# sta105/VIORB

Measured on AMD Instinct MI355X. Metric: frames/sec ORB extract+match+pose-opt, EuRoC 752x480, 1/2/4/8 GPUs, higher is better.
Workload: dtype u8

## Files before the change

### viorb_amd/csrc/orb_extractor.hip

```cpp
#include <hip/hip_runtime.h>
#include <stdlib.h>
#include <math.h>
#include <vector>
#include <string>
#include <algorithm>
#include "viorb_common.h"
#include "orb_math.h"
#include "octree_arrays.h"

namespace viorb {

static const int8_t kPatternHost[1024] = {
#include "orb_pattern.inc"
};

enum { MINB = 16, PATCH = 31, HALF_PATCH = 15, MAX_LEVELS = 16 };

struct LevelDev {
    int w, h, stride;
    uint32_t plane_off;
    int cell_base, ncells;
    int quota;
    int oct_w, oct_h;
    int n_ini;
// ... 151 lines not shown
    uint32_t v[RS2_TRIPS]; int at[RS2_TRIPS], gr[RS2_TRIPS], gc[RS2_TRIPS];
#pragma unroll
    for (int k = 0; k < RS2_TRIPS; k++) {
        const int i = threadIdx.x + 256 * k, ic = min(i, total - 1);
        const int r = ic / A.lds_pitch_dw, c = ic - r * A.lds_pitch_dw;
        at[k] = (i < total && c < ndw) ? i : -1;
        gr[k] = ys0 + r; gc[k] = xs0 + 4 * min(c, ndw - 1);
        v[k] = *reinterpret_cast<const uint32_t*>(src + (size_t)gr[k] * A.src_stride + gc[k]);
    }
    if (threadIdx.x < RS2_TW) s_xt[threadIdx.x] = tab; else if (threadIdx.x < RS2_TW + RS2_TH) s_yt[threadIdx.x - RS2_TW] = tab;
#pragma unroll
    for (int k = 0; k < RS2_TRIPS; k++) if (at[k] >= 0) s_tile[at[k]] = v[k];
    if (A.copy_dst) {
        uint8_t* cd = A.copy_dst + (size_t)b * A.copy_pitch;
#pragma unroll
        for (int k = 0; k < RS2_TRIPS; k++) if (at[k] >= 0) *reinterpret_cast<uint32_t*>(cd + (size_t)gr[k] * A.copy_stride + gc[k]) = v[k];
    }
    __syncthreads();
    const uint8_t* t8 = reinterpret_cast<const uint8_t*>(s_tile);
    const int xg = threadIdx.x & 15, r0 = threadIdx.x >> 4;
    int2 xt[4];
#pragma unroll
    for (int j = 0; j < 4; j++) xt[j] = s_xt[xg * 4 + j];
    uint8_t* dst = A.dst + (size_t)b * A.dst_pitch;
    const int pitch = A.lds_pitch_dw * 4;
#pragma unroll
    for (int half = 0; half < 2; half++) {
        const int r = r0 + 16 * half, dy = ty0 + r;
        if (dy >= A.dst_h) continue;
        const int2 yt = s_yt[r];
        const uint8_t* S0 = t8 + ((yt.x & 0xffff) - ys0) * pitch - xs0;
        const uint8_t* S1 = t8 + ((yt.x >> 16) - ys0) * pitch - xs0;
        const int b0 = yt.y & 0xffff, b1 = yt.y >> 16;
        uint32_t packed = 0;
#pragma unroll
        for (int j = 0; j < 4; j++) {
            const int sx0 = xt[j].x & 0xffff, sx1 = xt[j].x >> 16, a0 = xt[j].y & 0xffff, a1 = xt[j].y >> 16;
            const int h0 = S0[sx0] * a0 + S0[sx1] * a1;
            const int h1 = S1[sx0] * a0 + S1[sx1] * a1;
            const int val = (((b0 * (h0 >> 4)) >> 16) + ((b1 * (h1 >> 4)) >> 16) + 2) >> 2;
            packed |= (uint32_t)(val & 0xff) << (8 * j);
        }
        const int dxw = tx0 + xg * 4;
        if (dxw < A.dst_stride) *reinterpret_cast<uint32_t*>(dst + (size_t)dy * A.dst_stride + dxw) = packed;
    }
}

typedef unsigned short ushort2v __attribute__((ext_vector_type(2)));
__device__ __forceinline__ uint32_t dot2_u16(uint32_t a, uint32_t k, uint32_t c) {
    return __builtin_amdgcn_udot2(__builtin_bit_cast(ushort2v, a), __builtin_bit_cast(ushort2v, k), c, false);
}
#define RSS_LANES 32
#define RSS_PF 6
#define RSS_MAX_SRC_ROWS 60
struct ResizeStreamArgs {
    const uint8_t* planes; size_t frame_bytes;
    uint32_t src_off, dst_off;
    int src_stride, src_h, dst_stride, dst_w, dst_h;
    const int2* xtab; const int2* ytab; const uint2* etab; const int4* items;
};
struct __attribute__((packed, aligned(1))) rss_u8x8 { uint32_t lo, hi; };
__global__ __launch_bounds__(64) void k_resize_stream(ResizeStreamArgs A, XcdPlace PL) {
    int b, item;
    if (!xcd_place(PL, b, item)) return;
    const int4 t = A.items[item];
    const uint8_t* src = A.planes + (size_t)b * A.frame_bytes + A.src_off;
    uint8_t* dst = const_cast<uint8_t*>(A.planes) + (size_t)b * A.frame_bytes + A.dst_off;
    const int lane = threadIdx.x, hl = lane & (RSS_LANES - 1);
    const bool upper = lane >= RSS_LANES;
    const int Rb = t.z, y0A = t.y, y0B = t.y + Rb;
    const int rowsA = min(Rb, A.dst_h - y0A), rowsB = max(min(Rb, A.dst_h - y0B), 0);
    const int rsA = A.ytab[y0A].x & 0xffff, reA = A.ytab[y0A + rowsA - 1].x >> 16;
    const int rsB = rowsB > 0 ? A.ytab[min(y0B, A.dst_h - 1)].x & 0xffff : 0, reB = rowsB > 0 ? A.ytab[min(y0B + rowsB - 1, A.dst_h - 1)].x >> 16 : -1;
    const int ns = max(reA - rsA, reB - rsB) + 1;
    const int d = t.x + hl, sdw = A.dst_stride >> 2;
    uint32_t sel[4], aw[4]; int sxf = 0;
#pragma unroll
    for (int j = 0; j < 4; j++) {
        const int2 e = A.xtab[min(4 * d + j, A.dst_w - 1)];
        if (j == 0) sxf = e.x & 0xffff;
        sel[j] = (uint32_t)((e.x & 0xffff) - sxf) | ((uint32_t)((e.x >> 16) - sxf) << 16) | 0x0c000c00u;
        aw[j] = (uint32_t)e.y;
    }
    auto pack_entry = [&](int r0, int r1, int yb0, int nrows) {
        const int r = r0 + lane;
        const uint2 e = A.etab[min(r, A.src_h - 1)];
        const int y = (int)(e.x & 0x7fff) - yb0;
        const bool ok = r <= r1 && (e.x & 0x7fff) != 0x7fff && y >= 0 && y < nrows;
        return ok ? ((uint32_t)y | ((e.y & 0xfffu) << 7) | (((e.y >> 16) & 0xfffu) << 19) | ((e.x >> 15) << 31)) : 127u;
    };
    const uint32_t EA = pack_entry(rsA, reA, y0A, rowsA), EB = pack_entry(rsB, reB, y0B, rowsB);
    const uint8_t* pc = src + sxf;
    uint8_t* pd = dst + 4u * (uint32_t)min(d, sdw - 1);
    const bool col_ok = d < sdw;
    uint32_t lo[RSS_PF], hi[RSS_PF];
    auto request = [&](int i, uint32_t& l, uint32_t& h) {
        const uint32_t offA = __builtin_amdgcn_readfirstlane(min(rsA + i, A.src_h - 1) * A.src_stride), offB = __builtin_amdgcn_readfirstlane(min(rsB + i, A.src_h - 1) * A.src_stride);
        const rss_u8x8 v = *reinterpret_cast<const rss_u8x8*>(pc + (upper ? offB : offA));
        l = v.lo; h = v.hi;
    };
#pragma unroll
    for (int u = 0; u < RSS_PF; u++) request(u, lo[u], hi[u]);
    uint32_t hp[4] = {0, 0, 0, 0};
    for (int i0 = 0; i0 < ns; i0 += RSS_PF) {
#pragma unroll
        for (int u = 0; u < RSS_PF; u++) {
            const int i = i0 + u;
            uint32_t hc[4];
#pragma unroll
            for (int j = 0; j < 4; j++) {
                const uint32_t two = __builtin_amdgcn_perm(hi[u], lo[u], sel[j]);
                hc[j] = (dot2_u16(two, aw[j], 0u) & 0x7fff0u) << 5;
            }
            request(i + RSS_PF, lo[u], hi[u]);
            const uint32_t eA = __builtin_amdgcn_readlane(EA, i & 63), eB = __builtin_amdgcn_readlane(EB, i & 63);
            const uint32_t yrA = eA & 127u, yrB = eB & 127u;
            const bool emit = upper ? yrB < (uint32_t)rowsB : yrA < (uint32_t)rowsA;
            if (emit && col_ok) {
                const uint32_t b0 = upper ? (eB & (0xfffu << 7)) : (eA & (0xfffu << 7)), b1 = upper ? ((eB >> 12) & (0xfffu << 7)) : ((eA >> 12) & (0xfffu << 7));
                const uint32_t yoA = __builtin_amdgcn_readfirstlane((y0A + (int)yrA) * A.dst_stride), yoB = __builtin_amdgcn_readfirstlane((y0B + (int)yrB) * A.dst_stride);
                const uint32_t yo = upper ? yoB : yoA;
                uint32_t h0[4] = {hp[0], hp[1], hp[2], hp[3]};
                if ((int)(eA | eB) < 0) {
                    const bool same = upper ? (int)eB < 0 : (int)eA < 0;
#pragma unroll
                    for (int j = 0; j < 4; j++) h0[j] = same ? hc[j] : hp[j];
                }
                uint32_t v[4];
#pragma unroll
                for (int j = 0; j < 4; j++) {
                    const uint32_t t0 = (uint32_t)(((unsigned long long)h0[j] * b0) >> 32), t1 = (uint32_t)(((unsigned long long)hc[j] * b1) >> 32);
                    v[j] = (t0 + t1 + 2u) >> 2;
                }
                const uint32_t w01 = v[0] | (v[1] << 8), w23 = v[2] | (v[3] << 8);
                *reinterpret_cast<uint32_t*>(pd + yo) = w01 | (w23 << 16);
            }
#pragma unroll
            for (int j = 0; j < 4; j++) hp[j] = hc[j];
        }
    }
}

typedef short short2v __attribute__((ext_vector_type(2)));
__device__ __forceinline__ uint32_t pk_min16(uint32_t a, uint32_t b) {
    return __builtin_bit_cast(uint32_t, __builtin_elementwise_min(__builtin_bit_cast(short2v, a), __builtin_bit_cast(short2v, b)));
}
__device__ __forceinline__ uint32_t pk_max16(uint32_t a, uint32_t b) {
    return __builtin_bit_cast(uint32_t, __builtin_elementwise_max(__builtin_bit_cast(short2v, a), __builtin_bit_cast(short2v, b)));
}
__device__ __forceinline__ uint32_t pk_sub16(uint32_t a, uint32_t b) {
    return __builtin_bit_cast(uint32_t, __builtin_bit_cast(short2v, a) - __builtin_bit_cast(short2v, b));
}
__device__ __forceinline__ uint32_t swap16(uint32_t a) { return __builtin_amdgcn_alignbit(a, a, 16); }
__device__ __forceinline__ int fast_strength(const uint8_t* p, int pitch) {
    const uint32_t v = p[0], vv = v | (v << 16);
    uint32_t P[8];
    P[0] = pk_sub16(vv, (uint32_t)p[3 * pitch] | ((uint32_t)p[-3 * pitch] << 16));
    P[1] = pk_sub16(vv, (uint32_t)p[3 * pitch + 1] | ((uint32_t)p[-3 * pitch - 1] << 16));
    P[2] = pk_sub16(vv, (uint32_t)p[2 * pitch + 2] | ((uint32_t)p[-2 * pitch - 2] << 16));
    P[3] = pk_sub16(vv, (uint32_t)p[pitch + 3] | ((uint32_t)p[-pitch - 3] << 16));
    P[4] = pk_sub16(vv, (uint32_t)p[3] | ((uint32_t)p[-3] << 16));
    P[5] = pk_sub16(vv, (uint32_t)p[-pitch + 3] | ((uint32_t)p[pitch - 3] << 16));
    P[6] = pk_sub16(vv, (uint32_t)p[-2 * pitch + 2] | ((uint32_t)p[2 * pitch - 2] << 16));
    P[7] = pk_sub16(vv, (uint32_t)p[-3 * pitch + 1] | ((uint32_t)p[3 * pitch - 1] << 16));
    uint32_t S[8], lo2[8], hi2[8], lo4[8], hi4[8];
#pragma unroll
    for (int k = 0; k < 8; k++) S[k] = swap16(P[k]);
#pragma unroll
    for (int k = 0; k < 8; k++) { const uint32_t nx = k < 7 ? P[k + 1] : S[0]; lo2[k] = pk_min16(P[k], nx); hi2[k] = pk_max16(P[k], nx); }
#pragma unroll
    for (int k = 0; k < 8; k++) {
        const uint32_t nl = k < 6 ? lo2[k + 2] : swap16(lo2[k - 6]), nh = k < 6 ? hi2[k + 2] : swap16(hi2[k - 6]);
        lo4[k] = pk_min16(lo2[k], nl); hi4[k] = pk_max16(hi2[k], nh);
    }
    uint32_t A = 0x80008000u, B = 0x7fff7fffu;
#pragma unroll
    for (int k = 0; k < 8; k++) {
        const uint32_t nl = k < 4 ? lo4[k + 4] : swap16(lo4[k - 4]), nh = k < 4 ? hi4[k + 4] : swap16(hi4[k - 4]);
        A = pk_max16(A, pk_min16(pk_min16(lo4[k], nl), S[k]));
        B = pk_min16(B, pk_max16(pk_max16(hi4[k], nh), S[k]));
    }
    const int a = max((int)(short)(A & 0xffff), (int)(short)(A >> 16)), bq = min((int)(short)(B & 0xffff), (int)(short)(B >> 16));
    return max(a, -bq) - 1;
}

__device__ __forceinline__ int wave_inclusive_scan(int v) {
    v += __builtin_amdgcn_update_dpp(0, v, 0x111, 0xf, 0xf, false);
    v += __builtin_amdgcn_update_dpp(0, v, 0x112, 0xf, 0xf, false);
    v += __builtin_amdgcn_update_dpp(0, v, 0x114, 0xf, 0xf, false);
    v += __builtin_amdgcn_update_dpp(0, v, 0x118, 0xf, 0xf, false);
    v += __builtin_amdgcn_update_dpp(0, v, 0x142, 0xa, 0xf, false);
    v += __builtin_amdgcn_update_dpp(0, v, 0x143, 0xc, 0xf, false);
    return v;
}
__constant__ uint32_t c_rcp16[64];
#define FAST_FETCH_TRIPS 7
#define FAST_LAUNCHES 8
#define FAST_CELLS_PER_WAVE 2
__global__ __launch_bounds__(64) void k_fast_cells(const uint8_t* __restrict__ planes, size_t frame_bytes,
                                                   const LevelDev* __restrict__ lv,
                                                   const CellDesc* __restrict__ cells, int ini_th, int min_th,
                                                   uint32_t* __restrict__ slots, int slot_cap,
                                                   int* __restrict__ cell_cnt, int ncells_total,
                                                   int tile_bytes, int score_bytes, int list_cap, XcdPlace PL) {
    extern __shared__ uint32_t s_mem[];
    int img_b, item;
    if (!xcd_place(PL, img_b, item)) return;
    uint8_t* tile = reinterpret_cast<uint8_t*>(s_mem);
    uint8_t* sc = tile + tile_bytes;
    uint16_t* surv = reinterpret_cast<uint16_t*>(sc + score_bytes);
    uint16_t* corn = surv + list_cap;
    const int lane = threadIdx.x;
    const int cell0 = item * FAST_CELLS_PER_WAVE;
    const int ncell = min((int)FAST_CELLS_PER_WAVE, ncells_total - cell0);
    uint32_t v[FAST_FETCH_TRIPS];
    const uint8_t* img = planes + (size_t)img_b * frame_bytes;
    auto request_tile = [&](const CellDesc& cd) {
        const int pdw = cd.pitch >> 2;
// ... 748 lines not shown
            finish = true;
        } else if (live + n_to_expand * 3 > N) {
            int guard2 = 0;
            while (!finish && guard2++ < 4096) {
                const int prev2 = live;
                int m = 0;
                for (int base = first_new; base < nn; base += 64) {
                    const int i = base + lane;
                    bool want = false; SortKey key = 0;
                    if (i < nn) { const Node o = S.nd[i]; want = o.count > 1; key = ((SortKey)o.count << OctT<BIG>::KEY_SHIFT) | (SortKey)i; }
                    const unsigned long long bm = __ballot(want);
                    if (want) { const int pos = m + __popcll(bm & lanemask_lt(lane)); if (pos < sortcap) S.sortb[pos] = key; }
                    m += __popcll(bm);
                }
                if (m > sortcap) { overflow = true; m = sortcap; }
                int mp = 1; while (mp < m) mp <<= 1;
                for (int i = m + lane; i < mp; i += 64) S.sortb[i] = 0;
                WAVE_SYNC();
                oct_sort(S.sortb, mp, lane);
                const int nn1 = nn;
                int processed = 0;
                bool reached = false;
                for (int base = 0; base < m && !reached && !finish; base += 64) {
                    const int q = base + lane;
                    const bool valid = q < m;
                    const int i = valid ? (int)(S.sortb[mp - 1 - q] & 0xffff) : 0;
                    Node p; p.flags = OCT_DEAD; p.count = 0;
                    if (valid) p = S.nd[i];
                    if (__any(valid && p.count > OCT_LANE_LIMIT)) {
                        for (int l = 0; l < 64 && base + l < m; l++) {
                            if (nn1 + 4 * (processed + 1) > nodecap) { overflow = true; finish = true; break; }
                            const OctExpandResult r = oct_expand_wave(S, (int)(S.sortb[mp - 1 - (base + l)] & 0xffff), nn1 + 4 * processed, lane);
                            processed++; live += r.off - 1;
                            if (live >= N) { reached = true; break; }
                        }
                        continue;
                    }
                    const int mx = p.x0 + ((p.x1 - p.x0 + 1) >> 1), my = p.y0 + ((p.y1 - p.y0 + 1) >> 1);
                    unsigned long long lo = 0, hi = 0; int tc[4] = {0, 0, 0, 0};
                    if (valid) oct_lane_count(S, p, mx, my, lo, hi, tc);
                    const int inc = valid ? (tc[0] > 0) + (tc[1] > 0) + (tc[2] > 0) + (tc[3] > 0) - 1 : 0;
                    const int incl = wave_inclusive_scan(inc);
                    const unsigned long long mh = __ballot(valid && live + incl >= N);
                    const int nvalid = min(64, m - base);
                    int cut = mh ? __ffsll((long long)mh) - 1 : nvalid - 1;
                    const int fit = (nodecap - nn1) / 4 - processed;
                    if (fit < cut + 1) { overflow = true; finish = true; cut = fit - 1; }
                    if (valid && lane <= cut) oct_lane_scatter(S, p, i, nn1 + 4 * (processed + lane), mx, my, lo, hi, tc);
                    if (cut >= 0) { live += __shfl(incl, cut); processed += cut + 1; }
                    if (mh) reached = true;
                }
                nn = nn1 + 4 * processed;
                WAVE_SYNC();
                nn = oct_compact(S, nn, nn1, lane, first_new);
                if (live >= N || live == prev2) finish = true;
            }
        }
    }
    if (defer_nodes && overflow) {
        if (lane == 0) lvl_tot[b * nlevels + level] |= 0x40000000;
        return;
    }
    for (int base = 0; base < nn; base += 64) {
        const int i = base + lane;
        if (i < nn) {
            const Node o = S.nd[i];
            const Perm* pm = (o.flags & OCT_BUF) ? S.perm1 : S.perm0;
            uint32_t best = S.keys[pm[o.begin]];
            for (int k = 1; k < (int)o.count; k++) {
                const uint32_t key = S.keys[pm[o.begin + k]];
                if ((key >> 24) > (best >> 24)) best = key;
            }
            out[nn - 1 - i] = (best & 0xff000000u) | ((((best >> 12) & 0xfff) + MINB) << 12) | ((best & 0xfff) + MINB);
        }
    }
    if (lane == 0) {
        lvl_cnt[b * nlevels + level] = nn;
        if (overflow) status[b] = VIORB_ERR_CAPACITY;
    }
}

#define BS_LANES 32
#define BS_PF 6
__constant__ int c_gauss[7];
__global__ __launch_bounds__(64) void k_blur(const uint8_t* __restrict__ planes, uint8_t* __restrict__ blur,
                                             size_t frame_bytes, const LevelDev* __restrict__ lv,
                                             const int4* __restrict__ items, XcdPlace PL) {
    int b, item;
    if (!xcd_place(PL, b, item)) return;
    const int4 t = items[item];
    const LevelDev L = lv[t.x];
    const uint8_t* src = planes + (size_t)b * frame_bytes + L.plane_off;
    uint8_t* dst = blur + (size_t)b * frame_bytes + L.plane_off;
    const int lane = threadIdx.x, hl = lane & (BS_LANES - 1);
    const bool upper = lane >= BS_LANES;
    const int Rb = t.w, y0A = t.z, y0B = t.z + Rb;
    const int rows = upper ? min(Rb, L.h - y0B) : min(Rb, L.h - y0A);
    const int sdw = L.stride >> 2;
    const int d = t.y + hl;
    const int dlast = (L.w - 1) >> 2, m = (L.w - 1) & 3;
    const int dc = min(d, sdw - 1);
    const bool end_lane = hl == 0 || hl == BS_LANES - 1;
    const int dn = hl == 0 ? max(dc - 1, 0) : min(dc + 1, sdw - 1);
    const uint32_t selC = m == 0 ? 0x01020304u : m == 1 ? 0x03040504u : m == 2 ? 0x05060504u : 0x07060504u;
    const uint32_t selR = m == 0 ? 0x0c0c0c0cu : m == 1 ? 0x0c000102u : m == 2 ? 0x01020304u : 0x03040506u;
    const bool has_edge = t.y == 0 || t.y + BS_LANES > dlast - 1;
    const bool is_d0 = d == 0, is_dl = d == dlast, is_dl1 = d == dlast - 1;
    const uint32_t k0 = (uint32_t)c_gauss[0], k1 = (uint32_t)c_gauss[1], k2 = (uint32_t)c_gauss[2], k3 = (uint32_t)c_gauss[3];
    const uint32_t Ka = k0 | (k1 << 8) | (k2 << 16) | (k3 << 24), Kb = k2 | (k1 << 8) | (k0 << 16);
    const uint32_t K01 = k0 | (k1 << 16), K23 = k2 | (k3 << 16), K45 = k2 | (k1 << 16);
    const int nrow = Rb + 6;
    const uint8_t* pc = src + 4u * (uint32_t)dc;
    const uint8_t* pn = src + 4u * (uint32_t)(end_lane ? dn : dc);
    uint32_t cb[BS_PF], nb[BS_PF];
    auto request = [&](int i, uint32_t& c, uint32_t& n) {
        const int ii = min(i, nrow - 1);
        int ya = y0A + ii - 3, yb = y0B + ii - 3;
        ya = ya < 0 ? -ya : ya; ya = ya >= L.h ? 2 * L.h - 2 - ya : ya; ya = min(max(ya, 0), L.h - 1);
        yb = yb < 0 ? -yb : yb; yb = yb >= L.h ? 2 * L.h - 2 - yb : yb; yb = min(max(yb, 0), L.h - 1);
        const uint32_t offA = __builtin_amdgcn_readfirstlane(ya * L.stride), offB = __builtin_amdgcn_readfirstlane(yb * L.stride);
        const uint32_t off = upper ? offB : offA;
        c = *reinterpret_cast<const uint32_t*>(pc + off);
        n = *reinterpret_cast<const uint32_t*>(pn + off);
    };
#pragma unroll
    for (int u = 0; u < BS_PF; u++) request(u, cb[u], nb[u]);
    uint32_t P[6][4], hp[4] = {0, 0, 0, 0};
#pragma unroll
    for (int u = 0; u < 6; u++) { P[u][0] = P[u][1] = P[u][2] = P[u][3] = 0; }
    uint8_t* pd = dst + 4u * (uint32_t)min(d, sdw - 1);
    const bool col_ok = d < sdw;
    for (int i0 = 0; i0 < nrow; i0 += 6) {
#pragma unroll
        for (int u = 0; u < 6; u++) {
            const int i = i0 + u;
            uint32_t c = cb[u];
            uint32_t Lr = __builtin_amdgcn_update_dpp(c, c, 0x138, 0xf, 0xf, true);
            uint32_t Rr = __builtin_amdgcn_update_dpp(c, c, 0x130, 0xf, 0xf, true);
            Lr = hl == 0 ? nb[u] : Lr; Rr = hl == BS_LANES - 1 ? nb[u] : Rr;
            request(i + BS_PF, cb[u], nb[u]);
            if (has_edge) {
                const uint32_t Lf = __builtin_amdgcn_perm(Rr, c, 0x01020304u);
                const uint32_t Cf = __builtin_amdgcn_perm(c, Lr, selC), Rf = __builtin_amdgcn_perm(c, Lr, selR);
                const uint32_t Rf1 = __builtin_amdgcn_perm(Rr, c, selC);
                Lr = is_d0 ? Lf : Lr;
                Rr = is_dl ? Rf : (is_dl1 ? Rf1 : Rr);
                c = is_dl ? Cf : c;
            }
            uint32_t h[4];
            h[0] = __builtin_amdgcn_udot4(__builtin_amdgcn_alignbyte(c, Lr, 1), Ka, __builtin_amdgcn_udot4(__builtin_amdgcn_alignbyte(Rr, c, 1), Kb, 0u, false), false);
            h[1] = __builtin_amdgcn_udot4(__builtin_amdgcn_alignbyte(c, Lr, 2), Ka, __builtin_amdgcn_udot4(__builtin_amdgcn_alignbyte(Rr, c, 2), Kb, 0u, false), false);
            h[2] = __builtin_amdgcn_udot4(__builtin_amdgcn_alignbyte(c, Lr, 3), Ka, __builtin_amdgcn_udot4(__builtin_amdgcn_alignbyte(Rr, c, 3), Kb, 0u, false), false);
            h[3] = __builtin_amdgcn_udot4(c, Ka, __builtin_amdgcn_udot4(Rr, Kb, 0u, false), false);
            uint32_t a[4];
#pragma unroll
            for (int j = 0; j < 4; j++) {
                a[j] = dot2_u16(P[(u + 1) % 6][j], K01, 1u << 15);
                a[j] = dot2_u16(P[(u + 3) % 6][j], K23, a[j]);
                a[j] = dot2_u16(P[(u + 5) % 6][j], K45, a[j]);
                a[j] = __umul24(h[j], k0) + a[j];
                a[j] = min(a[j], 0x00ffffffu);
                P[u][j] = hp[j] | (h[j] << 16);
                hp[j] = h[j];
            }
            const int o = i - 6;
            const uint32_t yoA = __builtin_amdgcn_readfirstlane((y0A + o) * L.stride), yoB = __builtin_amdgcn_readfirstlane((y0B + o) * L.stride);
            if (o >= 0 && o < rows && col_ok) {
                const uint32_t lo = __builtin_amdgcn_perm(a[1], a[0], 0x0c0c0602u), hi = __builtin_amdgcn_perm(a[3], a[2], 0x0c0c0602u);
                *reinterpret_cast<uint32_t*>(pd + (upper ? yoB : yoA)) = lo | (hi << 16);
            }
        }
    }
}

__constant__ __attribute__((aligned(16))) uint32_t c_pattern[256];
__constant__ int c_umax[16];
__constant__ uint32_t c_orient_mask[256];
typedef uint32_t u32_unaligned __attribute__((aligned(1)));
#define DESC_WIN_HALF 18
#define DESC_WIN_ROWS 37
#define DESC_WIN_DW 10
#define DESC_WIN_TRIPS 6
__global__ __launch_bounds__(256) void k_orient_describe(const uint8_t* __restrict__ planes,
                                                         const uint8_t* __restrict__ blur, size_t frame_bytes,
                                                         const LevelDev* __restrict__ lv, int nlevels,
                                                         const uint32_t* __restrict__ lvl_kp, int kp_pitch,
                                                         const int* __restrict__ lvl_cnt,
                                                         viorb_keypoint* __restrict__ out_kp,
                                                         uint8_t* __restrict__ out_desc, int out_cap,
                                                         int* __restrict__ out_cnt, int* __restrict__ status, XcdPlace PL) {
    const int lane = threadIdx.x & 63;
    int b, item;
    if (!xcd_place(PL, b, item)) return;
    const int k = item * 4 + __builtin_amdgcn_readfirstlane(threadIdx.x >> 6);
    const int* cnt = lvl_cnt + b * nlevels;
    int level = -1, local = 0, total = 0;
    for (int l = 0; l < nlevels; l++) {
        const int c = cnt[l];
        if (level < 0 && k < total + c) { level = l; local = k - total; }
        total += c;
    }
    if (k == 0 && lane == 0) { out_cnt[b] = min(total, out_cap); if (total > out_cap) status[b] = VIORB_ERR_CAPACITY; }
    if (level < 0 || k >= out_cap) return;
    const LevelDev L = lv[level];
    const uint32_t key = lvl_kp[(size_t)b * kp_pitch + L.kp_off + local];
    const int cx = (int)(key & 0xfff), cy = (int)((key >> 12) & 0xfff), score = (int)(key >> 24);
    const uint8_t* img = planes + (size_t)b * frame_bytes + L.plane_off + (size_t)cy * L.stride + cx;
    __shared__ uint32_t s_win[4][DESC_WIN_ROWS * DESC_WIN_DW];
    uint32_t* win = s_win[threadIdx.x >> 6];
    const uint8_t* bim = blur + (size_t)b * frame_bytes + L.plane_off + (size_t)cy * L.stride + cx;
    uint32_t wv[DESC_WIN_TRIPS];
#pragma unroll
    for (int it = 0; it < DESC_WIN_TRIPS; it++) {
        const int i = min(lane + 64 * it, DESC_WIN_ROWS * DESC_WIN_DW - 1);
        const int wr = i / DESC_WIN_DW, wc = i - wr * DESC_WIN_DW;
        wv[it] = *reinterpret_cast<const u32_unaligned*>(bim + __mul24(wr - DESC_WIN_HALF, L.stride) - DESC_WIN_HALF + 4 * wc);
    }
    int m10 = 0, m01 = 0;
    {
        const int j = lane & 7, r8 = lane >> 3;
        const uint32_t wu = 0x03020100u + 0x04040404u * (uint32_t)j;
        const uint8_t* col = img - HALF_PATCH + 4 * j;
        uint32_t px[4]; int vv[4];
#pragma unroll
        for (int it = 0; it < 4; it++) {
            const int row = min(it * 8 + r8, PATCH - 1);
            vv[it] = row - HALF_PATCH;
            px[it] = *reinterpret_cast<const u32_unaligned*>(col + __mul24(vv[it], L.stride));
        }
#pragma unroll
        for (int it = 0; it < 4; it++) {
            const uint32_t q = px[it] & c_orient_mask[it * 64 + lane];
            const int s1 = (int)__builtin_amdgcn_udot4(q, 0x01010101u, 0u, false);
            const int su = (int)__builtin_amdgcn_udot4(q, wu, 0u, false);
            m10 += su - __mul24(HALF_PATCH, s1);
            m01 += __mul24(vv[it], s1);
        }
    }
    m10 = __builtin_amdgcn_readlane(wave_inclusive_scan(m10), 63); m01 = __builtin_amdgcn_readlane(wave_inclusive_scan(m01), 63);
    const float angle = fast_atan2_deg((float)m01, (float)m10);
    const float factor_pi = (float)(3.14159265358979323846 / 180.f);
    float sn, cs;
    sincos_f32(angle * factor_pi, &sn, &cs);
    const float a = cs, bb = sn;
#pragma unroll
    for (int it = 0; it < DESC_WIN_TRIPS; it++) {
        const int i = lane + 64 * it;
        if (i < DESC_WIN_ROWS * DESC_WIN_DW) win[i] = wv[it];
    }
    __builtin_amdgcn_fence(__ATOMIC_RELEASE, "wavefront"); __builtin_amdgcn_wave_barrier(); __builtin_amdgcn_fence(__ATOMIC_ACQUIRE, "wavefront");
    const uint8_t* w8 = reinterpret_cast<const uint8_t*>(win) + DESC_WIN_HALF * (DESC_WIN_DW * 4) + DESC_WIN_HALF;
    uint32_t nib = 0;
// ... 292 lines not shown
                    c.src_off = (uint32_t)(L.plane_off + (size_t)c.y0 * L.stride + (size_t)(c.x0 & ~3)); c.stride = L.stride;
                    if (c.cw < 7 || c.ch < 7) continue;
                    h->cells.push_back(c);
                    max_cw = std::max(max_cw, (int)c.cw); max_ch = std::max(max_ch, (int)c.ch);
                }
            }
        }
        L.ncells = (int)h->cells.size() - L.cell_base;
        L.n_ini = (L.oct_h > 0 && L.oct_w > 0) ? (int)roundf((float)L.oct_w / (float)L.oct_h) : 0;
        L.hx = L.n_ini > 0 ? (float)L.oct_w / (float)L.n_ini : 1.f;
        L.kp_off = kp_off;
        kp_off += std::max(L.quota, 4 * L.n_ini) + 4;
        L.xtab_off = (int)xtab.size(); L.ytab_off = (int)ytab.size();
        if (l > 0) {
            const int sw = h->lv[l - 1].w, sh = h->lv[l - 1].h;
            const double inv_sx = (double)L.w / sw, inv_sy = (double)L.h / sh;
            const double scale_x = 1. / inv_sx, scale_y = 1. / inv_sy;
            for (int dx = 0; dx < L.w; dx++) {
                float fx = (float)((dx + 0.5) * scale_x - 0.5);
                int sx = host_cv_floor(fx);
                fx -= sx;
                if (sx < 0) { fx = 0; sx = 0; }
                if (sx + 1 >= sw && sx >= sw - 1) { fx = 0; sx = sw - 1; }
                const int a0 = clampi(host_cv_round((double)((1.f - fx) * 2048)), -32768, 32767);
                const int a1 = clampi(host_cv_round((double)(fx * 2048)), -32768, 32767);
                const int sx1 = std::min(sx + 1, sw - 1);
                xtab.push_back(make_int2(sx | (sx1 << 16), (a0 & 0xffff) | (a1 << 16)));
            }
            for (int dy = 0; dy < L.h; dy++) {
                float fy = (float)((dy + 0.5) * scale_y - 0.5);
                int sy = host_cv_floor(fy);
                fy -= sy;
                const int b0 = clampi(host_cv_round((double)((1.f - fy) * 2048)), -32768, 32767);
                const int b1 = clampi(host_cv_round((double)(fy * 2048)), -32768, 32767);
                const int sy0 = clampi(sy, 0, sh - 1), sy1 = clampi(sy + 1, 0, sh - 1);
                ytab.push_back(make_int2(sy0 | (sy1 << 16), (b0 & 0xffff) | (b1 << 16)));
            }
            int maxdw = 1, maxrows = 1;
            const int2* xt = xtab.data() + L.xtab_off; const int2* yt = ytab.data() + L.ytab_off;
            for (int tx = 0; tx < L.w; tx += RS_TW) {
                const int x1 = std::min(tx + RS_TW, L.w) - 1;
                const int xs0 = (xt[tx].x & 0xffff) & ~3, xs1 = xt[x1].x >> 16;
                maxdw = std::max(maxdw, ((xs1 - xs0) >> 2) + 1);
            }
            for (int ty = 0; ty < L.h; ty += RS_TH) {
                const int y1 = std::min(ty + RS_TH, L.h) - 1;
                maxrows = std::max(maxrows, (yt[y1].x >> 16) - (yt[ty].x & 0xffff) + 1);
            }
            h->rs_pitch_dw[l] = maxdw; h->rs_rows[l] = maxrows;
            if ((size_t)maxdw * maxrows * 4 > 60000) { set_error("resize tile does not fit LDS (scale factor too large)"); return VIORB_ERR_UNSUPPORTED; }
            {
                h->rs2_off[l] = (int)h->rs2_tiles.size();
                int pdw = 1, prow = 1; bool cover = true; int next_x = 0, next_y = 0;
                const int gx2 = (L.w + RS2_TW - 1) / RS2_TW, gy2 = (L.h + RS2_TH - 1) / RS2_TH;
                for (int ty = 0; ty < gy2; ty++) {
                    const int y0t = ty * RS2_TH, y1t = std::min(y0t + RS2_TH, L.h) - 1;
                    const int ys0 = yt[y0t].x & 0xffff, ys1 = yt[y1t].x >> 16;
                    if (ys0 > next_y) cover = false;
                    next_y = std::max(next_y, ys1 + 1);
                    next_x = 0;
                    for (int tx = 0; tx < gx2; tx++) {
                        const int x0t = tx * RS2_TW, x1t = std::min(x0t + RS2_TW, L.w) - 1;
                        const int xs0 = (xt[x0t].x & 0xffff) & ~3, xs1 = xt[x1t].x >> 16;
                        if (xs0 > next_x) cover = false;
                        next_x = std::max(next_x, (xs1 | 3) + 1);
                        const int ndw = ((xs1 - xs0) >> 2) + 1, nrows = ys1 - ys0 + 1;
                        pdw = std::max(pdw, ndw); prow = std::max(prow, nrows);
                        h->rs2_tiles.push_back(make_int4(xs0, ndw, ys0, nrows));
                    }
                    if (next_x < sw) cover = false;
                }
                if (next_y < sh) cover = false;
                h->rs2_pitch_dw[l] = pdw;
                h->rs2_ok[l] = (prow <= 48 && pdw * prow <= 256 * RS2_TRIPS) ? 1 : 0;
                if (l == 1) h->rs2_copy_ok = cover && h->rs2_ok[1];
            }
            {
                static const bool no_stream = getenv("VIORB_RESIZE_TILES") != nullptr;
                bool ok = !no_stream && sw >= 8;
                h->rss_etab_off[l] = (int)h->rss_etab.size();
                std::vector<uint2> et(sh, make_uint2(0x7fffu, 0u));
                for (int dy = 0; dy < L.h && ok; dy++) {
                    const int sy0 = yt[dy].x & 0xffff, sy1 = yt[dy].x >> 16;
                    if ((sy1 != sy0 && sy1 != sy0 + 1) || et[sy1].x != 0x7fffu || dy >= 0x7fff) { ok = false; break; }
                    const int b0 = yt[dy].y & 0xffff, b1 = (yt[dy].y >> 16) & 0xffff;
                    if (b0 > 2048 || b1 > 2048) { ok = false; break; }
                    et[sy1] = make_uint2((uint32_t)dy | (sy1 == sy0 ? 0x8000u : 0u), (uint32_t)b0 | ((uint32_t)b1 << 16));
                }
                const int ndw = (L.w + 3) / 4;
                for (int dcol = 0; dcol < ndw && ok; dcol++) {
                    const int first = xt[std::min(4 * dcol, L.w - 1)].x & 0xffff;
                    for (int j = 0; j < 4; j++) {
                        const int2 e = xt[std::min(4 * dcol + j, L.w - 1)];
                        if ((e.x >> 16) - first > 7 || (e.x & 0xffff) < first || (e.y & 0xffff) > 2048 || ((e.y >> 16) & 0xffff) > 2048) ok = false;
                    }
                }
                h->rss_item_off[l] = (int)h->rss_items.size();
                if (ok) {
                    const double sy = (double)sh / L.h;
                    const int rbmax = std::max(1, std::min(100, (int)((RSS_MAX_SRC_ROWS - 2) / sy)));
                    const int nb = 2 * ((L.h + 2 * rbmax - 1) / (2 * rbmax)), rb = (L.h + nb - 1) / nb;
                    for (int k = 0; k < nb && ok; k++) {
                        const int ya = k * rb, yb = std::min(ya + rb, L.h) - 1;
                        if (ya <= yb && (yt[yb].x >> 16) - (yt[ya].x & 0xffff) + 1 > RSS_MAX_SRC_ROWS) ok = false;
                    }
                    for (int sx = 0; sx < ndw && ok; sx += RSS_LANES)
                        for (int k = 0; k < nb; k += 2)
                            if (k * rb < L.h) h->rss_items.push_back(make_int4(sx, k * rb, rb, 0));
                }
                if (!ok) h->rss_items.resize(h->rss_item_off[l]);
                h->rss_ok[l] = ok ? 1 : 0;
                h->rss_etab.insert(h->rss_etab.end(), et.begin(), et.end());
            }
        }
        {
            const int nb = 2 * ((L.h + 127) / 128), rb = (L.h + nb - 1) / nb, ndw = (L.w + 3) / 4;
            for (int sx = 0; sx < ndw; sx += BS_LANES)
                for (int k = 0; k < nb; k += 2) h->blur_tiles.push_back(make_int4(l, sx, k * rb, rb));
            if (L.w < 12 || L.h < 4) { set_error("level %d (%dx%d) too small for the blur", l, L.w, L.h); return VIORB_ERR_UNSUPPORTED; }
        }
    }
    h->frame_bytes = align_up(off, 256);
    h->kp_pitch = kp_off;
    h->out_cap = max_keypoints_for_size(h, w, hgt);
    const int ncells = (int)h->cells.size();
    if (ncells == 0) { set_error("image %dx%d too small for a FAST cell grid", w, hgt); return VIORB_ERR_UNSUPPORTED; }
    h->fast_tile_pitch = (int)align_up(max_cw + 3, 4) + 4;
    h->fast_tile_rows = max_ch;
    {
        int tb = 64 * FAST_FETCH_TRIPS * 4;
        for (const CellDesc& c : h->cells) tb = std::max(tb, c.pitch * c.ch);
        h->fast_tile_bytes = (int)align_up((size_t)tb, 16);
    }
    h->fast_score_bytes = (int)align_up((size_t)(max_cw - 6 + 2) * (max_ch - 6 + 2), 4);
    h->slot_cap = ((max_cw - 6 + 1) / 2) * ((max_ch - 6 + 1) / 2);
    h->fast_list_cap = (int)align_up((size_t)(max_cw - 6) * (max_ch - 6), 2);
    if (max_cw - 6 > 255 || max_ch - 6 > 255) { set_error("FAST cell larger than 255 px"); return VIORB_ERR_UNSUPPORTED; }
    {
        bool ok = true;
        for (const CellDesc& c : h->cells) ok = ok && ((c.x0 & 3) + c.cw <= 4 * F3_TPD - 4) && c.ch <= 4 * F3_TRIPS && c.cw - 6 + 2 <= F3_SP && c.ch - 6 + 2 <= F3_SROWS;
        static const bool force_v2 = getenv("VIORB_FAST_V2") != nullptr;
        h->fast_v3 = ok && !force_v2;
        h->fast3_tile_bytes = (int)align_up((size_t)(4 * ((max_ch + 3) / 4)) * F3_TP, 16);
        h->fast3_score_bytes = (int)align_up((size_t)(max_ch - 6 + 2) * F3_SP + 16, 16);
    }
    int maxq = 1; for (int l = 0; l < nl; l++) maxq = std::max(maxq, h->quota[l]);
    h->oct_ncap = 8192;
    h->oct_nodecap = 5 * maxq + 64;
    int sc = 1; while (sc < maxq + 8) sc <<= 1;
    h->oct_sortcap = sc;
    size_t oct_lds = (size_t)h->oct_ncap * 8 + (size_t)h->oct_nodecap * sizeof(OctNode) + (size_t)sc * 4;
    if (h->oct_nodecap > 65535) { set_error("per-level quota %d too large for the quadtree's 16-bit node indices", maxq); return VIORB_ERR_UNSUPPORTED; }
    h->oct_huge = oct_lds > 160 * 1024;
    if (!h->oct_huge && oct_lds > 64 * 1024 &&
        raise_dynamic_lds(reinterpret_cast<const void*>(k_octree<false>), oct_lds) != hipSuccess) {
        (void)hipGetLastError();
        h->oct_ncap = 4096;
        oct_lds = (size_t)h->oct_ncap * 8 + (size_t)h->oct_nodecap * sizeof(OctNode) + (size_t)sc * 4;
        if (oct_lds > 64 * 1024) { set_error("quadtree LDS (%zu B) exceeds the dynamic-LDS limit", oct_lds); return VIORB_ERR_UNSUPPORTED; }
    }

    if (!h->oct_huge) {
        const size_t lds_big = (size_t)h->oct_sortcap * 8 + (size_t)h->oct_nodecap * sizeof(OctNodeBig);
        if (lds_big > 160 * 1024) h->oct_huge = true;
        else if (lds_big > 64 * 1024) VIORB_HIP_TRY(raise_dynamic_lds(reinterpret_cast<const void*>(k_octree<true>), lds_big));
    }
    {
        const char* e = getenv("VIORB_OCT_TIERS");
        std::string spec = e ? e : "3:2048";
        h->oct_tiers.clear();
// ... 515 lines not shown
```

Before: 192,200.

## Streamline resize and blur inner loops with LDS emit table and incremental offsets

The streaming resize kernel now precomputes per-source-row emit weights into a shared-memory table and advances source and destination offsets incrementally, replacing per-iteration readlane/readfirstlane and row-index arithmetic. The same-row (sy1==sy0) case is no longer handled and is rejected on the host, so those levels fall back to another path. The blur kernel computes upper/lower row addresses from a base plus a uniform delta, moves the prefetch request later in the loop, and replaces the min-clamp and byte packing with v_sat_pk_u8_i16 saturation and incremental output offsets. The aim is to cut scalar/vector ALU work per row; the cost is an LDS write, a barrier and narrower eligibility for the streaming resize path.

```diff
diff --git a/viorb_amd/csrc/orb_extractor.hip b/viorb_amd/csrc/orb_extractor.hip
--- a/viorb_amd/csrc/orb_extractor.hip
+++ b/viorb_amd/csrc/orb_extractor.hip
@@ -257,58 +257,59 @@
         sel[j] = (uint32_t)((e.x & 0xffff) - sxf) | ((uint32_t)((e.x >> 16) - sxf) << 16) | 0x0c000c00u;
         aw[j] = (uint32_t)e.y;
     }
+    __shared__ uint2 s_emit[2][64];
     auto pack_entry = [&](int r0, int r1, int yb0, int nrows) {
         const int r = r0 + lane;
         const uint2 e = A.etab[min(r, A.src_h - 1)];
         const int y = (int)(e.x & 0x7fff) - yb0;
         const bool ok = r <= r1 && (e.x & 0x7fff) != 0x7fff && y >= 0 && y < nrows;
-        return ok ? ((uint32_t)y | ((e.y & 0xfffu) << 7) | (((e.y >> 16) & 0xfffu) << 19) | ((e.x >> 15) << 31)) : 127u;
+        return ok ? make_uint2(0x80000000u | ((e.y & 0xfffu) << 12), ((e.y >> 16) & 0xfffu) << 12) : make_uint2(0u, 0u);
     };
-    const uint32_t EA = pack_entry(rsA, reA, y0A, rowsA), EB = pack_entry(rsB, reB, y0B, rowsB);
-    const uint8_t* pc = src + sxf;
-    uint8_t* pd = dst + 4u * (uint32_t)min(d, sdw - 1);
-    const bool col_ok = d < sdw;
+    s_emit[0][lane] = pack_entry(rsA, reA, y0A, rowsA);
+    s_emit[1][lane] = pack_entry(rsB, reB, y0B, rowsB);
+    __syncthreads();
+    const uint2* em = s_emit[upper ? 1 : 0];
+    const uint32_t sstride = (uint32_t)A.src_stride, dstride = (uint32_t)A.dst_stride;
+    const uint32_t slast = (uint32_t)(A.src_h - 1) * sstride + (uint32_t)sxf;
+    uint32_t soff = (uint32_t)min(upper ? rsB : rsA, A.src_h - 1) * sstride + (uint32_t)sxf;
+    uint32_t doff = (uint32_t)(upper ? y0B : y0A) * dstride + 4u * (uint32_t)min(d, sdw - 1);
+    int colz = d < sdw ? 0 : (int)0x80000000u;
+    asm volatile("" : "+v"(colz));
     uint32_t lo[RSS_PF], hi[RSS_PF];
-    auto request = [&](int i, uint32_t& l, uint32_t& h) {
-        const uint32_t offA = __builtin_amdgcn_readfirstlane(min(rsA + i, A.src_h - 1) * A.src_stride), offB = __builtin_amdgcn_readfirstlane(min(rsB + i, A.src_h - 1) * A.src_stride);
-        const rss_u8x8 v = *reinterpret_cast<const rss_u8x8*>(pc + (upper ? offB : offA));
+    auto request = [&](uint32_t& l, uint32_t& h) {
+        const rss_u8x8 v = *reinterpret_cast<const rss_u8x8*>(src + soff);
         l = v.lo; h = v.hi;
+        soff = min(soff + sstride, slast);
     };
 #pragma unroll
-    for (int u = 0; u < RSS_PF; u++) request(u, lo[u], hi[u]);
+    for (int u = 0; u < RSS_PF; u++) request(lo[u], hi[u]);
     uint32_t hp[4] = {0, 0, 0, 0};
     for (int i0 = 0; i0 < ns; i0 += RSS_PF) {
+        uint2 E[RSS_PF];
+#pragma unroll
+        for (int u = 0; u < RSS_PF; u++) E[u] = em[i0 + u];
 #pragma unroll
         for (int u = 0; u < RSS_PF; u++) {
-            const int i = i0 + u;
+            const uint2 e = E[u];
             uint32_t hc[4];
 #pragma unroll
             for (int j = 0; j < 4; j++) {
                 const uint32_t two = __builtin_amdgcn_perm(hi[u], lo[u], sel[j]);
-                hc[j] = (dot2_u16(two, aw[j], 0u) & 0x7fff0u) << 5;
-            }
-            request(i + RSS_PF, lo[u], hi[u]);
-            const uint32_t eA = __builtin_amdgcn_readlane(EA, i & 63), eB = __builtin_amdgcn_readlane(EB, i & 63);
-            const uint32_t yrA = eA & 127u, yrB = eB & 127u;
-            const bool emit = upper ? yrB < (uint32_t)rowsB : yrA < (uint32_t)rowsA;
-            if (emit && col_ok) {
-                const uint32_t b0 = upper ? (eB & (0xfffu << 7)) : (eA & (0xfffu << 7)), b1 = upper ? ((eB >> 12) & (0xfffu << 7)) : ((eA >> 12) & (0xfffu << 7));
-                const uint32_t yoA = __builtin_amdgcn_readfirstlane((y0A + (int)yrA) * A.dst_stride), yoB = __builtin_amdgcn_readfirstlane((y0B + (int)yrB) * A.dst_stride);
-                const uint32_t yo = upper ? yoB : yoA;
-                uint32_t h0[4] = {hp[0], hp[1], hp[2], hp[3]};
-                if ((int)(eA | eB) < 0) {
-                    const bool same = upper ? (int)eB < 0 : (int)eA < 0;
-#pragma unroll
-                    for (int j = 0; j < 4; j++) h0[j] = same ? hc[j] : hp[j];
+                hc[j] = dot2_u16(two, aw[j], 0u) & 0x7fff0u;
+            }
+            request(lo[u], hi[u]);
+            if ((int)e.x < colz) {
+                uint32_t r[4];
+#pragma unroll
+                for (int j = 0; j < 4; j++) {
+                    const uint32_t t0 = (uint32_t)(((unsigned long long)(hp[j] & 0xffffffu) * (e.x & 0xffffffu)) >> 32);
+                    const uint32_t t1 = (uint32_t)(((unsigned long long)hc[j] * (e.y & 0xffffffu)) >> 32);
+                    r[j] = t0 + t1 + 2u;
                 }
-                uint32_t v[4];
-#pragma unroll
-                for (int j = 0; j < 4; j++) {
-                    const uint32_t t0 = (uint32_t)(((unsigned long long)h0[j] * b0) >> 32), t1 = (uint32_t)(((unsigned long long)hc[j] * b1) >> 32);
-                    v[j] = (t0 + t1 + 2u) >> 2;
-                }
-                const uint32_t w01 = v[0] | (v[1] << 8), w23 = v[2] | (v[3] << 8);
-                *reinterpret_cast<uint32_t*>(pd + yo) = w01 | (w23 << 16);
+                const uint32_t r02 = __builtin_amdgcn_perm(r[2], r[0], 0x05040100u), r13 = __builtin_amdgcn_perm(r[3], r[1], 0x05040100u);
+                const uint32_t v02 = (r02 >> 2) & 0x00ff00ffu, v13 = (r13 >> 2) & 0x00ff00ffu;
+                *reinterpret_cast<uint32_t*>(dst + doff) = v02 | (v13 << 8);
+                doff += dstride;
             }
 #pragma unroll
             for (int j = 0; j < 4; j++) hp[j] = hc[j];
@@ -1223,6 +1224,7 @@
 
 #define BS_LANES 32
 #define BS_PF 6
+#define BS_BIAS (1 << 23)
 __constant__ int c_gauss[7];
 __global__ __launch_bounds__(64) void k_blur(const uint8_t* __restrict__ planes, uint8_t* __restrict__ blur,
                                              size_t frame_bytes, const LevelDev* __restrict__ lv,
@@ -1245,32 +1247,36 @@
     const int dn = hl == 0 ? max(dc - 1, 0) : min(dc + 1, sdw - 1);
     const uint32_t selC = m == 0 ? 0x01020304u : m == 1 ? 0x03040504u : m == 2 ? 0x05060504u : 0x07060504u;
     const uint32_t selR = m == 0 ? 0x0c0c0c0cu : m == 1 ? 0x0c000102u : m == 2 ? 0x01020304u : 0x03040506u;
-    const bool has_edge = t.y == 0 || t.y + BS_LANES > dlast - 1;
+    const int has_edge = __builtin_amdgcn_readfirstlane(t.y == 0 || t.y + BS_LANES > dlast - 1 ? 1 : 0);
     const bool is_d0 = d == 0, is_dl = d == dlast, is_dl1 = d == dlast - 1;
     const uint32_t k0 = (uint32_t)c_gauss[0], k1 = (uint32_t)c_gauss[1], k2 = (uint32_t)c_gauss[2], k3 = (uint32_t)c_gauss[3];
     const uint32_t Ka = k0 | (k1 << 8) | (k2 << 16) | (k3 << 24), Kb = k2 | (k1 << 8) | (k0 << 16);
     const uint32_t K01 = k0 | (k1 << 16), K23 = k2 | (k3 << 16), K45 = k2 | (k1 << 16);
     const int nrow = Rb + 6;
-    const uint8_t* pc = src + 4u * (uint32_t)dc;
-    const uint8_t* pn = src + 4u * (uint32_t)(end_lane ? dn : dc);
+    int up = upper ? 1 : 0;
+    asm volatile("" : "+v"(up));
+    const int colc = 4 * dc + BS_BIAS, coln = 4 * (end_lane ? dn : dc) + BS_BIAS;
     uint32_t cb[BS_PF], nb[BS_PF];
     auto request = [&](int i, uint32_t& c, uint32_t& n) {
         const int ii = min(i, nrow - 1);
         int ya = y0A + ii - 3, yb = y0B + ii - 3;
         ya = ya < 0 ? -ya : ya; ya = ya >= L.h ? 2 * L.h - 2 - ya : ya; ya = min(max(ya, 0), L.h - 1);
         yb = yb < 0 ? -yb : yb; yb = yb >= L.h ? 2 * L.h - 2 - yb : yb; yb = min(max(yb, 0), L.h - 1);
-        const uint32_t offA = __builtin_amdgcn_readfirstlane(ya * L.stride), offB = __builtin_amdgcn_readfirstlane(yb * L.stride);
-        const uint32_t off = upper ? offB : offA;
-        c = *reinterpret_cast<const uint32_t*>(pc + off);
-        n = *reinterpret_cast<const uint32_t*>(pn + off);
+        const uint32_t offA = __builtin_amdgcn_readfirstlane(ya * L.stride);
+        const int delta = __builtin_amdgcn_readfirstlane((yb - ya) * L.stride);
+        const uint8_t* row = src + ((ptrdiff_t)offA - BS_BIAS);
+        c = *reinterpret_cast<const uint32_t*>(row + (uint32_t)(__mul24(up, delta) + colc));
+        n = *reinterpret_cast<const uint32_t*>(row + (uint32_t)(__mul24(up, delta) + coln));
     };
 #pragma unroll
     for (int u = 0; u < BS_PF; u++) request(u, cb[u], nb[u]);
     uint32_t P[6][4], hp[4] = {0, 0, 0, 0};
 #pragma unroll
     for (int u = 0; u < 6; u++) { P[u][0] = P[u][1] = P[u][2] = P[u][3] = 0; }
-    uint8_t* pd = dst + 4u * (uint32_t)min(d, sdw - 1);
-    const bool col_ok = d < sdw;
+    uint32_t doff = (uint32_t)(upper ? y0B : y0A) * (uint32_t)L.stride + 4u * (uint32_t)min(d, sdw - 1);
+    const uint32_t orows = d < sdw ? (uint32_t)max(rows, 0) : 0u;
+    uint32_t half = 1u << 15;
+    asm volatile("" : "+v"(half));
     for (int i0 = 0; i0 < nrow; i0 += 6) {
 #pragma unroll
         for (int u = 0; u < 6; u++) {
@@ -1279,7 +1285,6 @@
             uint32_t Lr = __builtin_amdgcn_update_dpp(c, c, 0x138, 0xf, 0xf, true);
             uint32_t Rr = __builtin_amdgcn_update_dpp(c, c, 0x130, 0xf, 0xf, true);
             Lr = hl == 0 ? nb[u] : Lr; Rr = hl == BS_LANES - 1 ? nb[u] : Rr;
-            request(i + BS_PF, cb[u], nb[u]);
             if (has_edge) {
                 const uint32_t Lf = __builtin_amdgcn_perm(Rr, c, 0x01020304u);
                 const uint32_t Cf = __builtin_amdgcn_perm(c, Lr, selC), Rf = __builtin_amdgcn_perm(c, Lr, selR);
@@ -1293,22 +1298,23 @@
             h[1] = __builtin_amdgcn_udot4(__builtin_amdgcn_alignbyte(c, Lr, 2), Ka, __builtin_amdgcn_udot4(__builtin_amdgcn_alignbyte(Rr, c, 2), Kb, 0u, false), false);
             h[2] = __builtin_amdgcn_udot4(__builtin_amdgcn_alignbyte(c, Lr, 3), Ka, __builtin_amdgcn_udot4(__builtin_amdgcn_alignbyte(Rr, c, 3), Kb, 0u, false), false);
             h[3] = __builtin_amdgcn_udot4(c, Ka, __builtin_amdgcn_udot4(Rr, Kb, 0u, false), false);
+            request(i + BS_PF, cb[u], nb[u]);
             uint32_t a[4];
 #pragma unroll
             for (int j = 0; j < 4; j++) {
-                a[j] = dot2_u16(P[(u + 1) % 6][j], K01, 1u << 15);
+                a[j] = dot2_u16(P[(u + 1) % 6][j], K01, half);
                 a[j] = dot2_u16(P[(u + 3) % 6][j], K23, a[j]);
                 a[j] = dot2_u16(P[(u + 5) % 6][j], K45, a[j]);
                 a[j] = __umul24(h[j], k0) + a[j];
-                a[j] = min(a[j], 0x00ffffffu);
                 P[u][j] = hp[j] | (h[j] << 16);
                 hp[j] = h[j];
             }
-            const int o = i - 6;
-            const uint32_t yoA = __builtin_amdgcn_readfirstlane((y0A + o) * L.stride), yoB = __builtin_amdgcn_readfirstlane((y0B + o) * L.stride);
-            if (o >= 0 && o < rows && col_ok) {
-                const uint32_t lo = __builtin_amdgcn_perm(a[1], a[0], 0x0c0c0602u), hi = __builtin_amdgcn_perm(a[3], a[2], 0x0c0c0602u);
-                *reinterpret_cast<uint32_t*>(pd + (upper ? yoB : yoA)) = lo | (hi << 16);
+            if ((uint32_t)(i - 6) < orows) {
+                uint32_t lo = __builtin_amdgcn_perm(a[1], a[0], 0x07060302u), hi = __builtin_amdgcn_perm(a[3], a[2], 0x07060302u);
+                asm("v_sat_pk_u8_i16 %0, %1" : "=v"(lo) : "v"(lo));
+                asm("v_sat_pk_u8_i16 %0, %1" : "=v"(hi) : "v"(hi));
+                doff += (uint32_t)L.stride;
+                *reinterpret_cast<uint32_t*>(dst - L.stride + doff) = lo | (hi << 16);
             }
         }
     }
@@ -1767,10 +1773,10 @@
                 std::vector<uint2> et(sh, make_uint2(0x7fffu, 0u));
                 for (int dy = 0; dy < L.h && ok; dy++) {
                     const int sy0 = yt[dy].x & 0xffff, sy1 = yt[dy].x >> 16;
-                    if ((sy1 != sy0 && sy1 != sy0 + 1) || et[sy1].x != 0x7fffu || dy >= 0x7fff) { ok = false; break; }
+                    if (sy1 != sy0 + 1 || et[sy1].x != 0x7fffu || dy >= 0x7fff) { ok = false; break; }
                     const int b0 = yt[dy].y & 0xffff, b1 = (yt[dy].y >> 16) & 0xffff;
                     if (b0 > 2048 || b1 > 2048) { ok = false; break; }
-                    et[sy1] = make_uint2((uint32_t)dy | (sy1 == sy0 ? 0x8000u : 0u), (uint32_t)b0 | ((uint32_t)b1 << 16));
+                    et[sy1] = make_uint2((uint32_t)dy, (uint32_t)b0 | ((uint32_t)b1 << 16));
                 }
                 const int ndw = (L.w + 3) / 4;
                 for (int dcol = 0; dcol < ndw && ok; dcol++) {
```

Measured after the change: 193,100, median of 6. No clear change (+0.5%).
